# hirofumi0810/tensorflow_end2end_speech_recognition

Hardware: AMD Instinct MI355X
Metric: acoustic frames/sec (train), TIMIT-shaped BLSTM-CTC (higher is better)
Workload: dtype bf16; 1 GPU; TIMIT 61-phone 5x256 BLSTM-CTC, B=16/GPU, D=120, C=62, seq_len~U{100..778}, dropout 0.2, rmsprop, train step; global_batch=16, parallelism=dp1, padded_to=own Tmax per rank

## Files before the change

### include/asr_hip.h

```cpp
#ifndef ASR_HIP_H_
#define ASR_HIP_H_

#include <stddef.h>
#include <stdint.h>

#ifdef __cplusplus
extern "C" {
#endif

typedef struct asr_handle asr_handle;
typedef void* asr_stream;

typedef enum {
  ASR_OK = 0,
  ASR_ERR_INVALID_ARG = -1,
  ASR_ERR_UNSUPPORTED = -2,
  ASR_ERR_HIP = -3,
  ASR_ERR_WORKSPACE = -4
} asr_status;

typedef enum { ASR_F32 = 0, ASR_BF16 = 1 } asr_dtype;

typedef enum {
  ASR_OPT_SGD = 0, ASR_OPT_MOMENTUM = 1, ASR_OPT_NESTEROV = 2, ASR_OPT_ADAGRAD = 3,
// ... 165 lines not shown
                    int Cout, int relu, int out_f32, void* out, asr_stream s);
int asr_conv3x4_bwd_data(asr_handle* h, const void* dy, int N, int H, int W, int Cout, const void* wt_bwd, int Cin,
                         float* dx, asr_stream s);
int asr_conv3x4_bwd_weight_bias(asr_handle* h, const void* x, const void* dy, int N, int H, int W, int Cin, int Cout,
                                float* dw, float* dbias, asr_stream s);
size_t asr_bn_workspace_bytes(long long M, int C);
int asr_bn_stats(asr_handle* h, const float* x, long long M, int C, float eps, float momentum, const float* avg_mean,
                 const float* avg_var, float* stats, void* ws, asr_stream s);
int asr_bn_apply(asr_handle* h, int out_dtype, const float* x, int N, int H, int W, int C, const float* mean,
                 const float* var, const float* gamma, const float* beta, float eps, int pool, void* out,
                 uint8_t* argmax, asr_stream s);
int asr_bn_bwd(asr_handle* h, int out_dtype, const float* dz, const uint8_t* argmax, int pool, const float* x, int N,
               int H, int W, int C, const float* stats, const float* gamma, int relu_gate, float* dgamma, float* dbeta,
               void* dx, void* ws, asr_stream s);
int asr_softmax_xent_soft(asr_handle* h, const float* logits, const float* targets, int rows, int C, float grad_scale,
                          float* row_loss, float* dlogits, asr_stream s);

int asr_lstm_prep_weights(asr_handle* h, int dtype, const float* kernel, const float* bias,
                          int Din, int H, void* wx_il, float* bias_il,
                          void* packed_fwd, void* packed_bwd, asr_stream s);
int asr_lstm_prep_layer(asr_handle* h, int dtype, int ndir, const float* const* vars, int Din, int ldk, int H,
                        void* wxT, void* wx_cat, float* bias_cat, void* packed_fwd, void* packed_bwd,
                        float* peep_out, asr_stream s);
int asr_lstm_grad_finish(asr_handle* h, int ndir, float* const* grads, int rows, int H, const float* dw_il,
                         const float* dpeep_dbias, int has_peep, asr_stream s);
int asr_gate_deinterleave(asr_handle* h, const float* in, int ld_in, float* out, int ld_out,
                          int rows, int H, asr_stream s);

int asr_lstm_fwd(asr_handle* h, int dtype, int T, int B, int H, int ndir,
                 const float* xproj, const void* wh_packed, const float* peep,
                 const int32_t* seq_len, float forget_bias, float cell_clip,
                 void* gates, void* hout, float* cs, float* c_final, float* h_final,
                 asr_stream s);

int asr_lstm_bwd(asr_handle* h, int dtype, int T, int B, int H, int ndir,
                 const float* dhout, const void* gates, const float* cs,
                 const void* wh_packed_bwd, const float* peep, const int32_t* seq_len,
                 const float* d_c_final, const float* d_h_final,
                 void* dgates, float* dpeep_dbias, float* dpeep_workspace, asr_stream s);
int asr_lstm_bwd_ex(asr_handle* h, int dtype, int T, int B, int H, int ndir,
                    const float* dhout, const void* gates, const float* cs,
                    const void* wh_packed_bwd, const float* peep, const int32_t* seq_len,
                    const float* d_c_final, const float* d_h_final, float clip_no_grad,
                    void* dgates, float* dpeep_dbias, float* dpeep_workspace, asr_stream s);

int asr_check_async_errors(asr_handle* h, unsigned* flags_out);
// ... 443 lines not shown
```

### tensorflow_end2end_speech_recognition_amd/_lib.py

```python
import ctypes as C
import os

_PKG = os.path.dirname(os.path.abspath(__file__))
LIB_PATH = os.path.join(_PKG, 'libasr_hip.so')

ASR_F32, ASR_BF16 = 0, 1
OPTIMIZER_IDS = {'sgd': 0, 'momentum': 1, 'nestrov': 2, 'adagrad': 3, 'adadelta': 4,
                 'rmsprop': 5, 'adam': 6}

_vp, _i, _f, _sz = C.c_void_p, C.c_int, C.c_float, C.c_size_t
_i64, _u64 = C.c_int64, C.c_uint64

SIGNATURES = {
    'asr_abi_version': (_i, []),
    'asr_create': (_i, [C.POINTER(_vp), _i]),
    'asr_create_ex': (_i, [C.POINTER(_vp), _i, _sz]),
    'asr_scratch_bytes': (_sz, [_vp]),
    'asr_destroy': (_i, [_vp]),
    'asr_set_xcd_skip': (_i, [_vp, _i]),
    'asr_set_gemm_tn_workgroups': (_i, [_vp, _i]),
    'asr_last_error_string': (C.c_char_p, [_vp]),
    'asr_device_info': (_i, [_vp, C.POINTER(_i), C.c_char_p, _i]),
    'asr_bt_to_tb': (_i, [_vp, _i, _vp, _vp, _i, _i, _i, _vp]),
    'asr_bt_to_tb_ld': (_i, [_vp, _i, _vp, _vp, _i, _i, _i, _i, _vp]),
    'asr_transpose2d': (_i, [_vp, _i, _vp, _i, _i, _i, _vp, _i, _vp]),
    'asr_cast_from_f32': (_i, [_vp, _i, _vp, _vp, _sz, _vp]),
    'asr_cast_to_f32': (_i, [_vp, _i, _vp, _vp, _sz, _vp]),
    'asr_apply_mask': (_i, [_vp, _i, _vp, _vp, _vp, _sz, _vp]),
    'asr_dropout_mask': (_i, [_vp, _vp, _sz, _f, _u64, _u64, _vp]),
    'asr_touch': (_i, [_vp, _vp, _sz, _vp]),
    'asr_dropout_apply': (_i, [_vp, _i, _vp, _vp, _sz, _f, _u64, _u64, _vp]),
    'asr_relu_bwd_drop': (_i, [_vp, _i, _vp, _vp, _sz, _f, _u64, _u64, _vp, _vp]),
    'asr_colsum': (_i, [_vp, _i, _vp, _i, _i, _i, _vp, _vp]),
    'asr_gemm': (_i, [_vp, _i, _i, _i, _i, _i, _i, _i, _vp, _i, _vp, _i, _vp, _i, _vp, _i, _vp]),
# ... 22 lines not shown
    'asr_relu_bwd_scaled': (_i, [_vp, _i, _vp, _vp, _sz, _f, _vp, _vp]),
    'asr_maxpool2x2_bwd': (_i, [_vp, _vp, _vp, _i, _i, _i, _i, _vp, _vp]),
    'asr_relu_bwd': (_i, [_vp, _i, _vp, _vp, _vp, _sz, _vp, _vp]),
    'asr_maxpool2x2_relu_bwd': (_i, [_vp, _i, _vp, _vp, _vp, _i, _i, _i, _i, _vp, _f, _u64, _u64, _i, _vp]),
    'asr_conv3x5_prep_weights': (_i, [_vp, _vp, _i, _i, _vp, _vp, _vp]),
    'asr_conv3x5_fwd': (_i, [_vp, _vp, _i, _i, _i, _i, _vp, _vp, _i, _i, _vp, _vp]),
    'asr_conv3x5_fwd_drop': (_i, [_vp, _vp, _i, _i, _i, _i, _vp, _vp, _i, _f, _u64, _u64, _vp, _vp]),
    'asr_conv3x5_bwd_data': (_i, [_vp, _vp, _i, _i, _i, _i, _vp, _i, _vp, _vp]),
    'asr_conv3x5_bwd_data_relu': (_i, [_vp, _vp, _i, _i, _i, _i, _vp, _i, _vp, _f, _u64, _u64, _i, _vp, _vp]),
    'asr_conv3x5_bwd_weight_bias': (_i, [_vp, _vp, _vp, _i, _i, _i, _i, _i, _vp, _vp, _vp]),
    'asr_maxpool3x1_fwd': (_i, [_vp, _i, _vp, _i, _i, _i, _i, _vp, _vp, _f, _u64, _u64, _i, _vp]),
    'asr_maxpool3x1_bwd': (_i, [_vp, _i, _vp, _vp, _i, _i, _i, _i, _vp, _vp]),
    'asr_conv3x4_prep_weights': (_i, [_vp, _vp, _i, _i, _vp, _vp, _vp]),
    'asr_conv3x4_fwd': (_i, [_vp, _vp, _i, _i, _i, _i, _vp, _vp, _i, _i, _i, _vp, _vp]),
    'asr_conv3x4_bwd_data': (_i, [_vp, _vp, _i, _i, _i, _i, _vp, _i, _vp, _vp]),
    'asr_conv3x4_bwd_weight_bias': (_i, [_vp, _vp, _vp, _i, _i, _i, _i, _i, _vp, _vp, _vp]),
    'asr_bn_workspace_bytes': (_sz, [_i64, _i]),
    'asr_bn_stats': (_i, [_vp, _vp, _i64, _i, _f, _f, _vp, _vp, _vp, _vp, _vp]),
    'asr_bn_apply': (_i, [_vp, _i, _vp, _i, _i, _i, _i, _vp, _vp, _vp, _vp, _f, _i, _vp, _vp, _vp]),
    'asr_bn_bwd': (_i, [_vp, _i, _vp, _vp, _i, _vp, _i, _i, _i, _i, _vp, _vp, _i, _vp, _vp, _vp, _vp, _vp]),
    'asr_softmax_xent_soft': (_i, [_vp, _vp, _vp, _i, _i, _f, _vp, _vp, _vp]),
    'asr_lstm_prep_weights': (_i, [_vp, _i, _vp, _vp, _i, _i, _vp, _vp, _vp, _vp, _vp]),
    'asr_lstm_prep_layer': (_i, [_vp, _i, _i, _vp, _i, _i, _i, _vp, _vp, _vp, _vp, _vp, _vp, _vp]),
    'asr_lstm_grad_finish': (_i, [_vp, _i, _vp, _i, _i, _vp, _vp, _i, _vp]),
    'asr_gate_deinterleave': (_i, [_vp, _vp, _i, _vp, _i, _i, _i, _vp]),
    'asr_lstm_fwd': (_i, [_vp, _i, _i, _i, _i, _i, _vp, _vp, _vp, _vp, _f, _f, _vp, _vp, _vp, _vp, _vp, _vp]),
    'asr_lstm_bwd': (_i, [_vp, _i, _i, _i, _i, _i, _vp, _vp, _vp, _vp, _vp, _vp, _vp, _vp, _vp, _vp,
                          _vp, _vp]),
    'asr_lstm_bwd_ex': (_i, [_vp, _i, _i, _i, _i, _i, _vp, _vp, _vp, _vp, _vp, _vp, _vp, _vp, _f, _vp, _vp,
                             _vp, _vp]),
    'asr_gru_fwd': (_i, [_vp, _i, _i, _i, _i, _vp, _vp, _vp, _vp, _vp, _i, _vp, _vp, _vp, _vp, _vp, _vp, _vp]),
    'asr_gru_bwd': (_i, [_vp, _i, _i, _i, _i, _vp, _vp, _vp, _vp, _vp, _vp, _vp, _vp, _vp, _i, _vp, _vp, _vp, _vp]),
    'asr_check_async_errors': (_i, [_vp, C.POINTER(C.c_uint)]),
    'asr_peek_async_errors': (_i, [_vp, _vp, _vp]),
    'asr_clear_async_errors': (_i, [_vp, _vp]),
    'asr_debug_set_lstm_flags': (_i, [_i]),
    'asr_debug_set_gru_persistent': (_i, [_i]),
    'asr_cluster_tile_groups': (_i, [_i, _i, _i, _i, C.POINTER(_i), C.POINTER(_i), _i]),
    'asr_recurrence_path_counts': (_i, [_vp, C.POINTER(C.c_ulonglong)]),
    'asr_reset_recurrence_path_counts': (_i, [_vp]),
    'asr_gru_kernel_counts': (_i, [_vp, C.POINTER(C.c_ulonglong)]),
    'asr_reset_gru_kernel_counts': (_i, [_vp]),
    'asr_lstm_kernel_counts': (_i, [_vp, C.POINTER(C.c_ulonglong), _i]),
    'asr_reset_lstm_kernel_counts': (_i, [_vp]),
    'asr_att_path_counts': (_i, [_vp, C.POINTER(C.c_ulonglong), _i]),
    'asr_reset_att_path_counts': (_i, [_vp]),
# ... 214 lines not shown
```

### tensorflow_end2end_speech_recognition_amd/csrc/lstm.hip

```cpp
#include "common.h"
#include <stdlib.h>

namespace {

template <typename T> struct LT;
template <> struct LT<float> {
  static constexpr int KV = 16;
  static constexpr int PAD = 4;
  typedef f32x4_t g4_t;
  static __device__ __forceinline__ g4_t pack(float a, float b, float c, float d) { return (g4_t){a, b, c, d}; }
  static __device__ __forceinline__ void unpack(const g4_t& v, float& a, float& b, float& c, float& d) {
    a = v[0]; b = v[1]; c = v[2]; d = v[3];
  }
  static __device__ __forceinline__ float cvt(float v) { return v; }
};
typedef __attribute__((ext_vector_type(4))) __bf16 bf16x4_t;
template <> struct LT<bf16_t> {
  static constexpr int KV = 32;
  static constexpr int PAD = 8;
  typedef bf16x4_t g4_t;
  static __device__ __forceinline__ g4_t pack(float a, float b, float c, float d) {
    return (g4_t){(__bf16)a, (__bf16)b, (__bf16)c, (__bf16)d};
  }
  static __device__ __forceinline__ void unpack(const g4_t& v, float& a, float& b, float& c, float& d) {
// ... 103 lines not shown
        const int k = ks * KV + kin;
        pf[(size_t)d * n_wh + i2] = Elem<T>::from_f32(wh[(size_t)k * G + q * H + ub * 16 + n]);
      }
      {
        const int KS = G / KV;
        const int ks = frag % KS;
        const int ub = frag / KS;
        const int kp = ks * KV + kin;
        pb[(size_t)d * n_wh + i2] = Elem<T>::from_f32(wh[(size_t)(ub * 16 + n) * G + (kp & 3) * H + (kp >> 2)]);
      }
      continue;
    }
    idx -= n_wh;
    if (idx < (size_t)G) {
      const int cp = (int)idx;
      bias_cat[(size_t)d * G + cp] = v.bias[d][(cp & 3) * H + (cp >> 2)];
      continue;
    }
    idx -= G;
    peep_out[(size_t)d * 3 * H + idx] = v.peep[d][idx / H][idx % H];
  }
}

struct GradVars { float* kernel[2]; float* bias[2]; float* peep[2][3]; };
__global__ void grad_finish_kernel(GradVars v, int ndir, int R, int H, const float* __restrict__ dw_il,
                                   const float* __restrict__ dpeep, int has_peep) {
  const int G = 4 * H;
  const size_t n_w = (size_t)R * G;
  const size_t per_dir = n_w + G + (has_peep ? (size_t)3 * H : 0);
  for (size_t gidx = blockIdx.x * (size_t)blockDim.x + threadIdx.x; gidx < per_dir * ndir;
       gidx += (size_t)gridDim.x * blockDim.x) {
    const int d = (int)(gidx / per_dir);
    size_t idx = gidx - (size_t)d * per_dir;
    if (idx < n_w) {
      const int r = (int)(idx / G), c = (int)(idx % G);
      const int q = c / H, j = c % H;
      v.kernel[d][idx] = dw_il[(size_t)d * n_w + (size_t)r * G + j * 4 + q];
      continue;
    }
    idx -= n_w;
    if (idx < (size_t)G) {
      v.bias[d][idx] = dpeep[((size_t)d * 7 + 3) * H + idx];
      continue;
    }
    idx -= G;
    v.peep[d][idx / H][idx % H] = dpeep[(size_t)d * 7 * H + idx];
// ... 559 lines not shown
    ASR_FAIL(h, ASR_ERR_INVALID_ARG, "asr_lstm_prep_layer: bad args (H=%d must be a multiple of 64, ldk=%d >= Din=%d)", H, ldk, Din);
  PrepVars v;
  memset(&v, 0, sizeof(v));
  for (int d = 0; d < ndir; ++d) {
    v.kernel[d] = vars[d * 5 + 0];
    v.bias[d] = vars[d * 5 + 1];
    for (int k = 0; k < 3; ++k) v.peep[d][k] = vars[d * 5 + 2 + k];
    if (!v.kernel[d] || !v.bias[d]) ASR_FAIL(h, ASR_ERR_INVALID_ARG, "asr_lstm_prep_layer: kernel / bias of direction %d missing", d);
    if (peep_out && (!v.peep[d][0] || !v.peep[d][1] || !v.peep[d][2]))
      ASR_FAIL(h, ASR_ERR_INVALID_ARG, "asr_lstm_prep_layer: peep_out given but a peephole vector of direction %d is missing", d);
  }
  const size_t total = (size_t)ndir * ((size_t)4 * H * ldk + (size_t)(Din + H + 1) * 4 * H + (peep_out ? 3 * H : 0));
  const int blocks = (int)((total + 255) / 256 < 4096 ? (total + 255) / 256 : 4096);
  if (dtype == ASR_F32)
    hipLaunchKernelGGL(prep_layer_kernel<float>, dim3(blocks), dim3(256), 0, (hipStream_t)s, v, ndir, Din, ldk, H,
                       (float*)wxT, (float*)wx_cat, bias_cat, (float*)packed_fwd, (float*)packed_bwd, peep_out);
  else
    hipLaunchKernelGGL(prep_layer_kernel<bf16_t>, dim3(blocks), dim3(256), 0, (hipStream_t)s, v, ndir, Din, ldk, H,
                       (bf16_t*)wxT, (bf16_t*)wx_cat, bias_cat, (bf16_t*)packed_fwd, (bf16_t*)packed_bwd, peep_out);
  ASR_CHECK_LAUNCH(h, "asr_lstm_prep_layer");
  return ASR_OK;
}

extern "C" int asr_lstm_grad_finish(asr_handle* h, int ndir, float* const* grads, int rows, int H,
                                    const float* dw_il, const float* dpeep_dbias, int has_peep, asr_stream s) {
  if (!h) return ASR_ERR_INVALID_ARG;
  if ((ndir != 1 && ndir != 2) || !grads || !dw_il || !dpeep_dbias || rows <= 0 || H <= 0)
    ASR_FAIL(h, ASR_ERR_INVALID_ARG, "asr_lstm_grad_finish: bad args");
  GradVars v;
  memset(&v, 0, sizeof(v));
  for (int d = 0; d < ndir; ++d) {
    v.kernel[d] = grads[d * 5 + 0];
    v.bias[d] = grads[d * 5 + 1];
    for (int k = 0; k < 3; ++k) v.peep[d][k] = grads[d * 5 + 2 + k];
    if (!v.kernel[d] || !v.bias[d] || (has_peep && (!v.peep[d][0] || !v.peep[d][1] || !v.peep[d][2])))
      ASR_FAIL(h, ASR_ERR_INVALID_ARG, "asr_lstm_grad_finish: a gradient pointer of direction %d is missing", d);
  }
  const size_t total = (size_t)ndir * ((size_t)(rows + 1) * 4 * H + (has_peep ? 3 * H : 0));
  const int blocks = (int)((total + 255) / 256 < 4096 ? (total + 255) / 256 : 4096);
  hipLaunchKernelGGL(grad_finish_kernel, dim3(blocks), dim3(256), 0, (hipStream_t)s, v, ndir, rows, H, dw_il,
                     dpeep_dbias, has_peep);
  ASR_CHECK_LAUNCH(h, "asr_lstm_grad_finish");
  return ASR_OK;
}

extern "C" int asr_lstm_fwd(asr_handle* h, int dtype, int T, int B, int H, int ndir,
// ... 105 lines not shown
```

### tensorflow_end2end_speech_recognition_amd/models/ctc/ctc.py

```python
import os as _os

import numpy as np
import torch

from ... import ops
from ..._lib import ASR_BF16, ASR_F32
from ...utils.io.labels.sparsetensor import dense_to_flat, sparse_to_flat
from ...utils.evaluation.edit_distance import compute_ler as _ler
from ...utils.parameter import ParamStore
from ..encoders.core.residual import check_residual, load_residual
from ..encoders.core.subsample import check_subsample, load_subsampled, shift_lengths
from ..encoders.load_encoder import load
from ..model_base import ModelBase


def truncated_normal(rng, stddev, shape):
    x = rng.normal(0.0, stddev, size=shape)
    bad = np.abs(x) > 2 * stddev
    while bad.any():
        x[bad] = rng.normal(0.0, stddev, size=int(bad.sum()))
        bad = np.abs(x) > 2 * stddev
    return x


# ... 67 lines not shown
        self.seed = seed

        self.bottleneck_dim = int(bottleneck_dim) if bottleneck_dim not in (None, 0) else None
        self.subsample_list = check_subsample(subsample_list, subsample_type, num_layers)
        self.subsample_type = subsample_type
        if any(self.subsample_list):
            load_subsampled(encoder_type)
        self.encoder_skip = check_residual(encoder_residual, encoder_dense_residual)
        if self.encoder_skip is not None:
            load_residual(encoder_type)
            if any(self.subsample_list):
                raise ValueError('skip connections join layers of one frame rate: not with a true subsample_list entry')
            if num_layers < 2:
                self.encoder_skip = None

        self.encoder = self._create_encoder(encoder_type, input_size, splice, num_stack, num_units, num_layers,
                                            lstm_impl, use_peephole, parameter_init, clip_activation)

        rng = np.random.RandomState(seed)
        self.store = ParamStore(self.device)
        enc_dim = self.encoder.build(self.store, input_size * num_stack * splice, rng)
        self._enc_dim = enc_dim
        self._head_imgs = None
        self._head_state = None
        self._declare_heads(rng, enc_dim, parameter_init)
        self.store.finalize()
        self._tape = None

    def _create_encoder(self, encoder_type, input_size, splice, num_stack, num_units, num_layers, lstm_impl,
                        use_peephole, parameter_init, clip_activation):
        if encoder_type in ['blstm', 'lstm']:
            if any(self.subsample_list):
                return load_subsampled(encoder_type)(
                    num_units=num_units, num_proj=self.num_proj, num_layers=num_layers,
                    lstm_impl=lstm_impl, use_peephole=use_peephole, parameter_init=parameter_init,
                    clip_activation=clip_activation, time_major=True, dtype=self._requested_dtype,
                    subsample_list=self.subsample_list, subsample_type=self.subsample_type)
            if self.encoder_skip is not None:
                return load_residual(encoder_type)(
                    num_units=num_units, num_proj=self.num_proj, num_layers=num_layers,
                    lstm_impl=lstm_impl, use_peephole=use_peephole, parameter_init=parameter_init,
                    clip_activation=clip_activation, time_major=True, dtype=self._requested_dtype,
                    dense=self.encoder_skip == 'dense')
            return load(encoder_type)(
                num_units=num_units, num_proj=self.num_proj, num_layers=num_layers,
                lstm_impl=lstm_impl, use_peephole=use_peephole, parameter_init=parameter_init,
# ... 68 lines not shown
            self._bn = None
            self._head_in = x_op
            return logits
        enc = x_op
        self._bn = None
        if self.bottleneck_dim:
            h = ops.gemm(x_op.view(T * Bp, E), sh['bottleneck/weights'], bias=self.store['bottleneck/biases'],
                         relu=True)
            mask = None
            hd = h
            if rng_state is not None:
                mask = ops.dropout_mask(h.shape, float(keep_prob), rng_state[0] + 11, rng_state[1], enc.device)
                hd = ops.apply_mask(h, mask)
            self._bn = dict(x=x_op, h=h, hd=hd, mask=mask)
            x_op, E = hd.view(T, Bp, self.bottleneck_dim), self.bottleneck_dim
        self._head_in = x_op
        logits = torch.empty((T, Bp, self.num_classes), dtype=torch.float32, device=enc.device)
        ops.gemm(x_op.view(T * Bp, E), sh[self.head_scope + '/weights'], bias=self.store[self.head_scope + '/biases'],
                 out=logits.view(T * Bp, self.num_classes))
        return logits

    def _refresh_head_shadow(self):
        if getattr(self, '_want_head_imgs', False):
            ops.ctc_head_prep(self.store[self.head_scope + '/weights'], out=self._head_imgs)
        sh = self.store.shadow(self.dtype)
        if sh is not self.store:
            for n in self.store.names:
                if n.endswith('/weights') and not n.startswith(('VGG', 'CNN', 'bridge', 'fc')):
                    sh[n]

    def _enc_operand(self):
        return self.encoder._out_op

    def create_placeholders(self):
        self.inputs_pl_list.append(Placeholder('input', np.float32,
                                               [None, None, self.input_size * self.num_stack * self.splice]))
        self.labels_pl_list.append(Placeholder('labels'))
        self.inputs_seq_len_pl_list.append(Placeholder('inputs_seq_len', np.int32, [None]))
        self.keep_prob_pl_list.append(Placeholder('keep_prob', np.float32))

    @staticmethod
    def _labels_to_flat(labels, batch_size):
        if isinstance(labels, (list, tuple)) and len(labels) == 3 and np.asarray(labels[0]).ndim == 2 \
                and np.asarray(labels[0]).shape[1] == 2 and np.asarray(labels[2]).shape == (2,):
            return sparse_to_flat(labels, batch_size)
        if torch.is_tensor(labels):
            labels = labels.cpu().numpy()
# ... 162 lines not shown
```

### tensorflow_end2end_speech_recognition_amd/models/encoders/core/blstm.py

```python
import collections
import os as _os

import numpy as np
import torch

from .... import ops
from ...._lib import ASR_F32
from ....utils.parameter import ParamStore
from . import rnn_util
from .rnn_util import LSTMLayer, LSTMPLayer, declare_lstm_vars, declare_lstmp_vars

WARM_BPTT = _os.environ.get('ASR_WARM_BPTT', '1') != '0'
ENC_HALVES = _os.environ.get('ASR_ENC_HALVES', '0') == '1'
PIPE_LANE = 6

LSTMStateTuple = collections.namedtuple('LSTMStateTuple', ('c', 'h'))

LSTM_IMPLS = ('BasicLSTMCell', 'LSTMCell', 'LSTMBlockCell', 'LSTMBlockFusedCell', 'CudnnLSTM')


class _RecurrentEncoderBase(object):
    ndir = 2
    scope_fmt = 'blstm_hidden%d'

    def __init__(self, num_units, num_proj, num_layers, lstm_impl, use_peephole, parameter_init,
                 clip_activation, time_major=True, name='lstm_encoder', dtype=ASR_F32, seed=0):
        assert num_proj != 0
        if lstm_impl not in LSTM_IMPLS:
            raise IndexError('lstm_impl is "BasicLSTMCell" or "LSTMCell" or "LSTMBlockCell" or '
                             '"LSTMBlockFusedCell" or "CudnnLSTM".')
        self.num_units = num_units
        self.num_proj = num_proj if lstm_impl == 'LSTMCell' else None
        if self.num_proj is not None and type(self).__name__ not in ('BLSTMEncoder', 'LSTMEncoder', 'VGGBLSTMEncoder',
                                                                     'VGGLSTMEncoder', 'MultitaskBLSTMEncoder',
                                                                     'MultitaskLSTMEncoder', 'CLDNNEncoder'):
            raise ValueError('LSTMCell projection layers (num_proj) are implemented for the blstm / lstm / vgg_* / '
# ... 4 lines not shown
        self.parameter_init = parameter_init
        self.clip_activation = None if lstm_impl == 'BasicLSTMCell' else clip_activation
        self.time_major = time_major
        self.name = name
        self.dtype = ops.dtype_id(dtype)
        self.layer_dtype = self.dtype
        if self.num_proj is not None:
            self.dtype = ASR_F32
        self.seed = seed
        self.layers = None
        self.store = None
        self.scope_prefix = ''
        self.num_layers_sub = None
        self.grad_ready_hook = None
        self.side_extra = None
        self.side_extra_event = None
        self.defer_top_dropout = False
        self._top_deferred, self._top_drop = False, None
        self.want_f32_outputs = True
        self.halves = ENC_HALVES
        self.layers_b = None
        self._split = 0
        self._rows = None

    def build(self, store, input_dim, rng, scope_prefix=''):
        self.store = store
        self.scope_prefix = scope_prefix
        self.layers = []
        din = input_dim
        H = self.num_units
        if self.num_proj is not None:
            P = int(self.num_proj)
            for i in range(1, self.num_layers + 1):
                bases = self._declare_projected(store, i, din, P, rng)
                self.layers.append(LSTMPLayer(store, bases, din, H, P, self.use_peephole, 1.0, self.clip_activation,
                                              dtype=self.layer_dtype))
                din = self.ndir * P
            self.output_dim = self.ndir * P
            return self.output_dim
        for i in range(1, self.num_layers + 1):
            bases = self._declare(store, i, din, rng)
            self.layers.append(LSTMLayer(store, bases, din, H, self.use_peephole, 1.0,
                                         self.clip_activation))
            din = self.ndir * H
        self.output_dim = self.ndir * H
        return self.output_dim
# ... 18 lines not shown
        self._ensure_built(inputs)
        lens_host = getattr(self, '_lens_host', None)
        self._lens_host = None
        if self.num_proj is not None:
            return self._call_projected(inputs, inputs_seq_len, keep_prob, is_training, drop_masks, rng_state)
        B, T, _ = inputs.shape
        self.pad_b = (-B) % 16
        if self.pad_b:
            inputs = torch.cat([inputs, inputs.new_zeros(self.pad_b, T, inputs.shape[2])], 0)
            inputs_seq_len = torch.cat([inputs_seq_len, inputs_seq_len.new_zeros(self.pad_b)], 0)
        self.batch = B
        seq_len = inputs_seq_len.to(torch.int32).contiguous()
        Tt, Bp = T, inputs.shape[0]
        D = inputs.shape[2]
        ldk0 = (D + 63) // 64 * 64 if self.dtype != ASR_F32 else D

        if rng_state is None and drop_masks is None and is_training and keep_prob is not None and keep_prob < 1.0:
            self._dropout_calls = getattr(self, '_dropout_calls', 0) + 1
            rng_state = (self.seed, self._dropout_calls << 40)

        def rs_of(li):
            return (rng_state[0], rng_state[1] + li * (1 << 32)) if rng_state is not None else None

        preps, ready_w, ready_m = [], [], []
        with ops.side_lane(inputs.device):
            fold = self.side_extra is not None and len(self.layers) >= 2
            self.side_extra_event = None
            for li, layer in enumerate(self.layers):
                preps.append(layer.prepare(inputs.device, self.dtype, Tt, Bp, 1.0, False, None, None,
                                           ldk=ldk0 if li == 0 else None))
                if fold and li + 1 == len(self.layers):
                    self.side_extra()
                ready_w.append(ops.stream_event())
            if self.side_extra is not None and not fold:
                self.side_extra()
                self.side_extra_event = ops.stream_event()
            for li, layer in enumerate(self.layers):
                dm = drop_masks[li] if drop_masks is not None else None
                preps[li]['mask'] = layer.make_mask(inputs.device, Tt, Bp, keep_prob, is_training, rs_of(li), dm)
                ready_m.append(ops.stream_event())
        self._split = self._split_rows(Bp) if drop_masks is None else 0
        self._top_deferred, self._top_drop = False, None
        plans = rnn_util.row_plans(lens_host, B, Tt, Bp, self._split) if (self.dtype != ASR_F32 and inputs.is_cuda) \
            else None
        self._rows = None
        if plans is not None:
            self._rows = [(t, int(p.size)) for t, p in zip(ops.upload_ints(inputs.device, plans), plans)]
        if self._split:
            x, finals = self._forward_halves(inputs, seq_len, preps, ready_w, ready_m, keep_prob, is_training, ldk0)
            return self._finish_call(x, finals, seq_len, B)
        x = ops.bt_to_tb(inputs.contiguous(), self.dtype, ld=ldk0)
        final = None
        finals = []
        for li, layer in enumerate(self.layers):
            if not rnn_util.FORK_ONCE or li == 0:
                ops.wait_event(ready_w[li])
            elif li == 1:
                ops.wait_event(ready_w[-1])
            top = li + 1 == len(self.layers)
            mk = preps[li]['mask']
            defer = top and self.defer_top_dropout and self.num_layers_sub is None and (mk is None or isinstance(mk, tuple))
            x, final = layer.forward(x, seq_len, self.dtype, keep_prob, is_training, prep=preps[li],
                                     mask_event=ready_m[li], rows=self._rows[0] if self._rows else None,
                                     defer_mask=defer or self._connects(li))
            if defer:
                self._top_deferred, self._top_drop = True, mk
            x = self._connect(li, x, mk, seq_len)
            finals.append(final)
            if self.num_layers_sub is not None and li + 1 == self.num_layers_sub:
                self._out_sub_op, self._final_sub_ch = x, final
        return self._finish_call(x, finals, seq_len, B)

    def _connects(self, li):
        return False

    def _connect(self, li, x, mask, seq_len):
        return x

    def _finish_call(self, x, finals, seq_len, B):
        self.seq_len_padded = seq_len
        self._out_op = x
        out = ops.cast_to_f32(x) if (x.dtype != torch.float32 and self.want_f32_outputs) else x
        self._out_tm = out
        cf, hf = finals[-1]
        self._final_ch = (cf, hf)
        self._finals = finals
        final_state = self._state_tuple(finals, len(finals))
        out_user = out[:, :B]
        if not self.time_major:
            out_user = out_user.transpose(0, 1)
        return out_user, final_state

    def _split_rows(self, Bp):
        tiles = Bp // 16
# ... 185 lines not shown
```

### tensorflow_end2end_speech_recognition_amd/ops.py

```python
import ctypes as C
import math
import os
import time as _time

import numpy as np
import torch

from . import _lib
from ._lib import ASR_BF16, ASR_F32

TORCH_DTYPE = {ASR_F32: torch.float32, ASR_BF16: torch.bfloat16}


def dtype_id(dtype):
    if dtype in (ASR_F32, 'f32', 'fp32', 'float32', torch.float32):
        return ASR_F32
    if dtype in (ASR_BF16, 'bf16', 'bfloat16', torch.bfloat16):
        return ASR_BF16
    raise ValueError('dtype must be f32 or bf16, got %r' % (dtype,))


_lane = 0
_side = {}

# ... 937 lines not shown
                   pb=torch.empty((H * 4 * H,), dtype=tdt, device=dev))
    h.check(h.lib.asr_lstm_prep_weights(h.h, dtype, _p(kernel), _p(bias), din, H, _p(out['wx_il']),
                                        _p(out['bias_il']), _p(out['pf']), _p(out['pb']), _s()),
            'asr_lstm_prep_weights')
    return out


def gate_deinterleave(src, dst, H):
    h = _h(src)
    h.check(h.lib.asr_gate_deinterleave(h.h, C.c_void_p(src.data_ptr()), src.stride(0),
                                        C.c_void_p(dst.data_ptr()), dst.stride(0), src.shape[0], H, _s()),
            'asr_gate_deinterleave')
    return dst


def _ptr_table(rows):
    flat = []
    for r in rows:
        r = list(r) + [None] * (5 - len(r))
        flat.extend(t.data_ptr() if t is not None else None for t in r)
    return (C.c_void_p * len(flat))(*flat)


def lstm_prep_layer(variables, din, H, dtype, ldk=None):
    k0 = variables[0][0]
    h = _h(k0)
    ndir = len(variables)
    ldk = din if ldk is None else int(ldk)
    for v in variables:
        _chk(v[0], torch.float32, 'kernel')
        if v[0].shape != (din + H, 4 * H):
            raise ValueError('kernel must be [Din+H,4H]')
    has_peep = len(variables[0]) >= 5 and variables[0][2] is not None
    dev, tdt = k0.device, TORCH_DTYPE[dtype]
    out = dict(wxT=torch.empty((ndir * 4 * H, ldk), dtype=tdt, device=dev),
               wx_cat=torch.empty((din, ndir * 4 * H), dtype=tdt, device=dev),
               bias=torch.empty((ndir * 4 * H,), dtype=torch.float32, device=dev),
               whf=torch.empty((ndir, H * 4 * H), dtype=tdt, device=dev),
               whb=torch.empty((ndir, H * 4 * H), dtype=tdt, device=dev),
               peep=torch.empty((ndir, 3, H), dtype=torch.float32, device=dev) if has_peep else None)
    h.check(h.lib.asr_lstm_prep_layer(h.h, dtype, ndir, _ptr_table(variables), din, ldk, H, _p(out['wxT']),
                                      _p(out['wx_cat']), _p(out['bias']), _p(out['whf']), _p(out['whb']),
                                      _p(out['peep']), _s()), 'asr_lstm_prep_layer')
    return out


def lstm_grad_finish(grads, dw_il, dpeep, H):
    h = _h(dw_il)
    ndir, rows, _ = dw_il.shape
    has_peep = len(grads[0]) >= 5 and grads[0][2] is not None
    h.check(h.lib.asr_lstm_grad_finish(h.h, ndir, _ptr_table(grads), rows, H, _p(dw_il), _p(dpeep),
                                       1 if has_peep else 0, _s()), 'asr_lstm_grad_finish')


LSTM_UNITS = (64, 128, 192, 256, 320, 512)


def lstm_units_supported(H):
    return int(H) in LSTM_UNITS


def lstm_fwd(xproj, wh_packed, peep, seq_len, H, ndir, dtype, forget_bias=1.0, cell_clip=0.0,
             want_final=True):
    h = _h(xproj)
    _chk(xproj, torch.float32, 'xproj')
    _chk(seq_len, torch.int32, 'seq_len')
    T, B, G = xproj.shape
# ... 2000 lines not shown
```

### tensorflow_end2end_speech_recognition_amd/utils/parameter.py

```python
import numpy as np
import torch

from .. import ops
from .._lib import ASR_BF16


class ParamStore(object):
    def __init__(self, device):
        self.device = device
        self._specs = []
        self._index = {}
        self.flat = None
        self.grad = None
        self.views = {}
        self.gviews = {}
        self.finalized = False
        self._shadow = None
        self._shadow_dirty = True
        self._backup = None
        self.perturbed = False

    def declare(self, name, shape, init):
        if self.finalized:
            raise RuntimeError('ParamStore already finalized; cannot declare %s' % name)
        if name in self._index:
            raise ValueError('variable %s already exists' % name)
        init = np.asarray(init, dtype=np.float32).reshape(shape)
        self._index[name] = len(self._specs)
        self._specs.append((name, tuple(int(s) for s in shape), init))

    def finalize(self):
        offs = [0]
        starts = []
        pos = 0
        for name, shape, _ in self._specs:
            n = int(np.prod(shape)) if len(shape) else 1
            starts.append(pos)
            pos += (n + 15) // 16 * 16
            offs.append(pos)
        self.total = pos
        host = np.zeros(self.total, dtype=np.float32)
        for (name, shape, init), st in zip(self._specs, starts):
            host[st:st + init.size] = init.ravel()
# ... 11 lines not shown
        self.finalized = True
        self._shadow_dirty = True

    def __getitem__(self, name):
        return self.views[name]

    def g(self, name):
        return self.gviews[name]

    def bucket(self, first, last):
        i0, i1 = self._index[first], self._index[last]
        if i1 < i0:
            raise ValueError('bucket: %s is declared after %s' % (first, last))
        off = self.offsets_host[i0:i1 + 2] - self.offsets_host[i0]
        start, end = int(self.offsets_host[i0]), int(self.offsets_host[i1 + 1])
        return dict(start=start, end=end, names=self.names[i0:i1 + 1], grad=self.grad[start:end],
                    plan=ops.ClipPlan(off, self.flat.device))

    def num_params(self):
        return int(sum(int(np.prod(s[1])) if len(s[1]) else 1 for s in self._specs))

    def mark_dirty(self):
        self._shadow_dirty = True

    def shadow(self, dtype):
        if dtype != ASR_BF16:
            return self
        if self._shadow is None:
            self._shadow = _Shadow(self)
        if self._shadow_dirty:
            self._shadow.invalidate()
            self._shadow_dirty = False
        return self._shadow

    def perturb(self, std, seed, offset):
        if self.perturbed:
            raise RuntimeError('ParamStore.perturb: the previous perturbation was not restored')
        if self._backup is None:
            self._backup = torch.empty_like(self.flat)
        ops.weight_noise_perturb(self.flat, self._backup, std, seed, offset)
        self.perturbed = True
        self.mark_dirty()

    def restore(self):
        if not self.perturbed:
            return
# ... 95 lines not shown
```

Measured before the change: 766,000 frames/s.

## Batch LSTM weight prep into one multi-layer kernel and cache images by version

Adds a grouped prep kernel that packs the input, recurrent and bias/peephole weight images for all LSTM layers in a single launch instead of one launch per layer on a side stream. The encoder now caches these prepared images and the CTC head image, keyed on the parameter store's tensor version and a mutation epoch, so they are rebuilt only when the weights change. In training the optimizer updates the weights every step, so each step still runs one fused prep call, issued on the main stream rather than overlapped on the side lane. This trades the removed launches and side-stream events for losing that overlap, and adds key-tracking complexity.

```diff
diff --git a/include/asr_hip.h b/include/asr_hip.h
--- a/include/asr_hip.h
+++ b/include/asr_hip.h
@@ -211,6 +211,16 @@
 int asr_lstm_prep_layer(asr_handle* h, int dtype, int ndir, const float* const* vars, int Din, int ldk, int H,
                         void* wxT, void* wx_cat, float* bias_cat, void* packed_fwd, void* packed_bwd,
                         float* peep_out, asr_stream s);
+typedef struct asr_lstm_prep_desc {
+  int ndir;
+  const float* const* vars;
+  int Din, ldk, H;
+  void *wxT, *wx_cat;
+  float* bias_cat;
+  void *packed_fwd, *packed_bwd;
+  float* peep_out;
+} asr_lstm_prep_desc;
+int asr_lstm_prep_layers(asr_handle* h, int dtype, int nlayers, const asr_lstm_prep_desc* layers, asr_stream s);
 int asr_lstm_grad_finish(asr_handle* h, int ndir, float* const* grads, int rows, int H, const float* dw_il,
                          const float* dpeep_dbias, int has_peep, asr_stream s);
 int asr_gate_deinterleave(asr_handle* h, const float* in, int ld_in, float* out, int ld_out,
diff --git a/tensorflow_end2end_speech_recognition_amd/_lib.py b/tensorflow_end2end_speech_recognition_amd/_lib.py
--- a/tensorflow_end2end_speech_recognition_amd/_lib.py
+++ b/tensorflow_end2end_speech_recognition_amd/_lib.py
@@ -10,6 +10,11 @@
 
 _vp, _i, _f, _sz = C.c_void_p, C.c_int, C.c_float, C.c_size_t
 _i64, _u64 = C.c_int64, C.c_uint64
+
+class LstmPrepDesc(C.Structure):
+    _fields_ = [('ndir', _i), ('vars', _vp), ('Din', _i), ('ldk', _i), ('H', _i), ('wxT', _vp), ('wx_cat', _vp),
+                ('bias_cat', _vp), ('packed_fwd', _vp), ('packed_bwd', _vp), ('peep_out', _vp)]
+
 
 SIGNATURES = {
     'asr_abi_version': (_i, []),
@@ -78,6 +83,7 @@
     'asr_softmax_xent_soft': (_i, [_vp, _vp, _vp, _i, _i, _f, _vp, _vp, _vp]),
     'asr_lstm_prep_weights': (_i, [_vp, _i, _vp, _vp, _i, _i, _vp, _vp, _vp, _vp, _vp]),
     'asr_lstm_prep_layer': (_i, [_vp, _i, _i, _vp, _i, _i, _i, _vp, _vp, _vp, _vp, _vp, _vp, _vp]),
+    'asr_lstm_prep_layers': (_i, [_vp, _i, _i, _vp, _vp]),
     'asr_lstm_grad_finish': (_i, [_vp, _i, _vp, _i, _i, _vp, _vp, _i, _vp]),
     'asr_gate_deinterleave': (_i, [_vp, _vp, _i, _vp, _i, _i, _i, _vp]),
     'asr_lstm_fwd': (_i, [_vp, _i, _i, _i, _i, _i, _vp, _vp, _vp, _vp, _f, _f, _vp, _vp, _vp, _vp, _vp, _vp]),
diff --git a/tensorflow_end2end_speech_recognition_amd/csrc/lstm.hip b/tensorflow_end2end_speech_recognition_amd/csrc/lstm.hip
--- a/tensorflow_end2end_speech_recognition_amd/csrc/lstm.hip
+++ b/tensorflow_end2end_speech_recognition_amd/csrc/lstm.hip
@@ -149,6 +149,109 @@
   }
 }
 
+constexpr int PREP_MAX_LAYERS = 16;
+struct PrepLayer {
+  PrepVars v;
+  void *wxT, *wx_cat;
+  float* bias_cat;
+  void *pf, *pb;
+  float* peep_out;
+  int ndir, Din, ldk, H;
+  int block0, upd, nX, nB, nF;
+};
+struct PrepGroup { PrepLayer l[PREP_MAX_LAYERS]; int n; };
+static_assert(sizeof(PrepGroup) <= 4096, "PrepGroup must fit the kernel argument segment");
+
+template <typename T>
+__global__ __launch_bounds__(256) void prep_layers_kernel(PrepGroup g) {
+  constexpr int KV = LT<T>::KV;
+  constexpr int E = 16 / sizeof(T);
+  static_assert(KV == 4 * E, "a fragment is four row groups of E elements");
+  constexpr int SX = 129, SB = 136, SF = 40;
+  __shared__ float tile[32 * SX];
+  int li = 0;
+  while (li + 1 < g.n && (int)blockIdx.x >= g.l[li + 1].block0) ++li;
+  const PrepLayer& L = g.l[li];
+  const int H = L.H, G = 4 * H, Din = L.Din, ldk = L.ldk, ndir = L.ndir, HT = H / 32;
+  int u = (int)blockIdx.x - L.block0;
+  const int d = u / L.upd;
+  u -= d * L.upd;
+  const float* __restrict__ kernel = L.v.kernel[d];
+  const float* __restrict__ wh = kernel + (size_t)Din * G;
+  const size_t n_wh = (size_t)H * G;
+  const int t = threadIdx.x;
+  if (u < L.nX) {
+    const int r0 = (u / HT) * 32, j0 = (u % HT) * 32;
+#pragma unroll
+    for (int i = 0; i < 16; ++i) {
+      const int e = t + 256 * i, rl = e >> 7, c = e & 127, q = c >> 5, jj = c & 31, r = r0 + rl;
+      tile[rl * SX + jj * 4 + q] = r < Din ? kernel[(size_t)r * G + q * H + j0 + jj] : 0.f;
+    }
+    __syncthreads();
+    T* __restrict__ wx_cat = (T*)L.wx_cat;
+    T* __restrict__ wxT = (T*)L.wxT;
+#pragma unroll
+    for (int i = 0; i < 16; ++i) {
+      const int e = t + 256 * i, rl = e >> 7, cpl = e & 127, r = r0 + rl;
+      if (r < Din) wx_cat[(size_t)r * ndir * G + (size_t)d * G + j0 * 4 + cpl] = Elem<T>::from_f32(tile[rl * SX + cpl]);
+    }
+#pragma unroll
+    for (int i = 0; i < 16; ++i) {
+      const int e = t + 256 * i, cpl = e >> 5, rl = e & 31, r = r0 + rl;
+      if (r < ldk) wxT[((size_t)d * G + j0 * 4 + cpl) * ldk + r] = Elem<T>::from_f32(tile[rl * SX + cpl]);
+    }
+    return;
+  }
+  u -= L.nX;
+  if (u < L.nB) {
+    const int ub = u / HT, j0 = (u % HT) * 32;
+#pragma unroll
+    for (int i = 0; i < 8; ++i) {
+      const int e = t + 256 * i, n = e >> 7, c = e & 127, q = c >> 5, jj = c & 31;
+      tile[n * SB + jj * 4 + q] = wh[(size_t)(ub * 16 + n) * G + q * H + j0 + jj];
+    }
+    __syncthreads();
+    T* __restrict__ pb = (T*)L.pb + (size_t)d * n_wh + (size_t)ub * 16 * G + (size_t)64 * j0;
+#pragma unroll
+    for (int i = 0; i < 8; ++i) {
+      const int o = t + 256 * i, e = o % E, n = (o / E) & 15, rg = (o / (16 * E)) & 3, ksl = o / (64 * E);
+      pb[o] = Elem<T>::from_f32(tile[n * SB + ksl * KV + rg * E + e]);
+    }
+    return;
+  }
+  u -= L.nB;
+  if (u < L.nF) {
+    const int k0 = (u / (4 * HT)) * 32, q = (u % (4 * HT)) / HT, u0 = (u % HT) * 32;
+#pragma unroll
+    for (int i = 0; i < 4; ++i) {
+      const int e = t + 256 * i, kl = e >> 5, cl = e & 31;
+      tile[kl * SF + cl] = wh[(size_t)(k0 + kl) * G + q * H + u0 + cl];
+    }
+    __syncthreads();
+    T* __restrict__ pf = (T*)L.pf + (size_t)d * n_wh;
+#pragma unroll
+    for (int i = 0; i < 4; ++i) {
+      const int o4 = t + 256 * i, ubl = o4 >> 9, o = o4 & 511;
+      const int e = o % E, n = (o / E) & 15, rg = (o / (16 * E)) & 3, ksl = o / (64 * E);
+      const int ub = u0 / 16 + ubl, kl = ksl * KV + rg * E + e;
+      pf[((size_t)(ub * 4 + q) * H + k0) * 16 + o] = Elem<T>::from_f32(tile[kl * SF + ubl * 16 + n]);
+    }
+    return;
+  }
+  u -= L.nF;
+  if (u < G / 256) {
+    const int cp = u * 256 + t;
+    L.bias_cat[(size_t)d * G + cp] = L.v.bias[d][(cp & 3) * H + (cp >> 2)];
+    return;
+  }
+  const int idx = (u - G / 256) * 256 + t;
+  if (idx < 3 * H) {
+    const int k = idx / H;
+    const float* p = k == 0 ? L.v.peep[d][0] : k == 1 ? L.v.peep[d][1] : L.v.peep[d][2];
+    L.peep_out[(size_t)d * 3 * H + idx] = p[idx - k * H];
+  }
+}
+
 struct GradVars { float* kernel[2]; float* bias[2]; float* peep[2][3]; };
 __global__ void grad_finish_kernel(GradVars v, int ndir, int R, int H, const float* __restrict__ dw_il,
                                    const float* __restrict__ dpeep, int has_peep) {
@@ -754,6 +857,57 @@
   return ASR_OK;
 }
 
+extern "C" int asr_lstm_prep_layers(asr_handle* h, int dtype, int nlayers, const asr_lstm_prep_desc* layers,
+                                    asr_stream s) {
+  if (!h) return ASR_ERR_INVALID_ARG;
+  if (!asr_dtype_ok(dtype) || nlayers < 0 || (nlayers && !layers))
+    ASR_FAIL(h, ASR_ERR_INVALID_ARG, "asr_lstm_prep_layers: bad args");
+  for (int i = 0; i < nlayers; ++i) {
+    const asr_lstm_prep_desc& L = layers[i];
+    if ((L.ndir != 1 && L.ndir != 2) || !L.vars || !L.wxT || !L.wx_cat || !L.bias_cat || !L.packed_fwd ||
+        !L.packed_bwd || L.Din <= 0 || L.ldk < L.Din || L.H <= 0 || L.H % 64)
+      ASR_FAIL(h, ASR_ERR_INVALID_ARG, "asr_lstm_prep_layers: layer %d: H=%d must be a multiple of 64, ldk=%d >= Din=%d", i,
+               L.H, L.ldk, L.Din);
+    for (int d = 0; d < L.ndir; ++d) {
+      if (!L.vars[d * 5] || !L.vars[d * 5 + 1])
+        ASR_FAIL(h, ASR_ERR_INVALID_ARG, "asr_lstm_prep_layers: kernel / bias of layer %d, direction %d missing", i, d);
+      if (L.peep_out && (!L.vars[d * 5 + 2] || !L.vars[d * 5 + 3] || !L.vars[d * 5 + 4]))
+        ASR_FAIL(h, ASR_ERR_INVALID_ARG, "asr_lstm_prep_layers: peep_out given but a peephole vector of layer %d, direction %d is missing", i, d);
+    }
+  }
+  for (int i0 = 0; i0 < nlayers; i0 += PREP_MAX_LAYERS) {
+    PrepGroup g;
+    memset(&g, 0, sizeof(g));
+    g.n = nlayers - i0 < PREP_MAX_LAYERS ? nlayers - i0 : PREP_MAX_LAYERS;
+    long long blocks = 0;
+    for (int i = 0; i < g.n; ++i) {
+      const asr_lstm_prep_desc& L = layers[i0 + i];
+      PrepLayer& P = g.l[i];
+      for (int d = 0; d < L.ndir; ++d) {
+        P.v.kernel[d] = L.vars[d * 5 + 0];
+        P.v.bias[d] = L.vars[d * 5 + 1];
+        for (int k = 0; k < 3; ++k) P.v.peep[d][k] = L.vars[d * 5 + 2 + k];
+      }
+      P.wxT = L.wxT, P.wx_cat = L.wx_cat, P.bias_cat = L.bias_cat, P.pf = L.packed_fwd, P.pb = L.packed_bwd;
+      P.peep_out = L.peep_out;
+      P.ndir = L.ndir, P.Din = L.Din, P.ldk = L.ldk, P.H = L.H;
+      const long long HT = L.H / 32;
+      const long long nX = ((long long)L.ldk + 31) / 32 * HT, nB = (L.H / 16) * HT, nF = HT * HT * 4;
+      const long long upd = nX + nB + nF + 4 * L.H / 256 + (L.peep_out ? (3 * L.H + 255) / 256 : 0);
+      if (blocks + L.ndir * upd > 0x7fffffffLL)
+        ASR_FAIL(h, ASR_ERR_INVALID_ARG, "asr_lstm_prep_layers: layer %d: too many units for one grid", i0 + i);
+      P.block0 = (int)blocks, P.upd = (int)upd, P.nX = (int)nX, P.nB = (int)nB, P.nF = (int)nF;
+      blocks += L.ndir * upd;
+    }
+    if (dtype == ASR_F32)
+      hipLaunchKernelGGL(prep_layers_kernel<float>, dim3((unsigned)blocks), dim3(256), 0, (hipStream_t)s, g);
+    else
+      hipLaunchKernelGGL(prep_layers_kernel<bf16_t>, dim3((unsigned)blocks), dim3(256), 0, (hipStream_t)s, g);
+    ASR_CHECK_LAUNCH(h, "asr_lstm_prep_layers");
+  }
+  return ASR_OK;
+}
+
 extern "C" int asr_lstm_grad_finish(asr_handle* h, int ndir, float* const* grads, int rows, int H,
                                     const float* dw_il, const float* dpeep_dbias, int has_peep, asr_stream s) {
   if (!h) return ASR_ERR_INVALID_ARG;
diff --git a/tensorflow_end2end_speech_recognition_amd/models/ctc/ctc.py b/tensorflow_end2end_speech_recognition_amd/models/ctc/ctc.py
--- a/tensorflow_end2end_speech_recognition_amd/models/ctc/ctc.py
+++ b/tensorflow_end2end_speech_recognition_amd/models/ctc/ctc.py
@@ -113,6 +113,7 @@
         enc_dim = self.encoder.build(self.store, input_size * num_stack * splice, rng)
         self._enc_dim = enc_dim
         self._head_imgs = None
+        self._head_key = None
         self._head_state = None
         self._declare_heads(rng, enc_dim, parameter_init)
         self.store.finalize()
@@ -227,7 +228,10 @@
 
     def _refresh_head_shadow(self):
         if getattr(self, '_want_head_imgs', False):
-            ops.ctc_head_prep(self.store[self.head_scope + '/weights'], out=self._head_imgs)
+            key = self.store.image_key() if getattr(self.encoder, 'weight_images', False) else None
+            if key is None or key != self._head_key:
+                ops.ctc_head_prep(self.store[self.head_scope + '/weights'], out=self._head_imgs)
+                self._head_key = key
         sh = self.store.shadow(self.dtype)
         if sh is not self.store:
             for n in self.store.names:
diff --git a/tensorflow_end2end_speech_recognition_amd/models/encoders/core/blstm.py b/tensorflow_end2end_speech_recognition_amd/models/encoders/core/blstm.py
--- a/tensorflow_end2end_speech_recognition_amd/models/encoders/core/blstm.py
+++ b/tensorflow_end2end_speech_recognition_amd/models/encoders/core/blstm.py
@@ -12,6 +12,7 @@
 
 WARM_BPTT = _os.environ.get('ASR_WARM_BPTT', '1') != '0'
 ENC_HALVES = _os.environ.get('ASR_ENC_HALVES', '0') == '1'
+WEIGHT_IMAGES = _os.environ.get('ASR_WEIGHT_IMAGES', '1') != '0'
 PIPE_LANE = 6
 
 LSTMStateTuple = collections.namedtuple('LSTMStateTuple', ('c', 'h'))
@@ -62,6 +63,8 @@
         self.layers_b = None
         self._split = 0
         self._rows = None
+        self.weight_images = WEIGHT_IMAGES
+        self._images, self._image_key = None, None
 
     def build(self, store, input_dim, rng, scope_prefix=''):
         self.store = store
@@ -126,23 +129,12 @@
         def rs_of(li):
             return (rng_state[0], rng_state[1] + li * (1 << 32)) if rng_state is not None else None
 
-        preps, ready_w, ready_m = [], [], []
-        with ops.side_lane(inputs.device):
-            fold = self.side_extra is not None and len(self.layers) >= 2
-            self.side_extra_event = None
-            for li, layer in enumerate(self.layers):
-                preps.append(layer.prepare(inputs.device, self.dtype, Tt, Bp, 1.0, False, None, None,
-                                           ldk=ldk0 if li == 0 else None))
-                if fold and li + 1 == len(self.layers):
-                    self.side_extra()
-                ready_w.append(ops.stream_event())
-            if self.side_extra is not None and not fold:
-                self.side_extra()
-                self.side_extra_event = ops.stream_event()
-            for li, layer in enumerate(self.layers):
-                dm = drop_masks[li] if drop_masks is not None else None
-                preps[li]['mask'] = layer.make_mask(inputs.device, Tt, Bp, keep_prob, is_training, rs_of(li), dm)
-                ready_m.append(ops.stream_event())
+        if self.weight_images:
+            preps, ready_w, ready_m = self._cached_preps(inputs.device, ldk0, Tt, Bp, keep_prob, is_training, rs_of,
+                                                         drop_masks)
+        else:
+            preps, ready_w, ready_m = self._side_preps(inputs.device, ldk0, Tt, Bp, keep_prob, is_training, rs_of,
+                                                       drop_masks)
         self._split = self._split_rows(Bp) if drop_masks is None else 0
         self._top_deferred, self._top_drop = False, None
         plans = rnn_util.row_plans(lens_host, B, Tt, Bp, self._split) if (self.dtype != ASR_F32 and inputs.is_cuda) \
@@ -174,6 +166,45 @@
             if self.num_layers_sub is not None and li + 1 == self.num_layers_sub:
                 self._out_sub_op, self._final_sub_ch = x, final
         return self._finish_call(x, finals, seq_len, B)
+
+    def _cached_preps(self, device, ldk0, Tt, Bp, keep_prob, is_training, rs_of, drop_masks):
+        key = self.store.image_key() + (self.dtype, ldk0)
+        if key != self._image_key:
+            self._images = ops.lstm_prep_layers(
+                [dict(variables=layer._vars(self.store.__getitem__), din=layer.din, H=layer.H, dtype=self.dtype,
+                      ldk=ldk0 if li == 0 else None) for li, layer in enumerate(self.layers)])
+            self._image_key = key
+        self.side_extra_event = None
+        if self.side_extra is not None:
+            self.side_extra()
+        preps, ready_m = [], []
+        for li, layer in enumerate(self.layers):
+            dm = drop_masks[li] if drop_masks is not None else None
+            w = dict(self._images[li])
+            w['mask'] = layer.make_mask(device, Tt, Bp, keep_prob, is_training, rs_of(li), dm)
+            preps.append(w)
+            ready_m.append(ops.stream_event() if torch.is_tensor(w['mask']) and w['mask'].is_cuda else None)
+        return preps, [None] * len(self.layers), ready_m
+
+    def _side_preps(self, device, ldk0, Tt, Bp, keep_prob, is_training, rs_of, drop_masks):
+        preps, ready_w, ready_m = [], [], []
+        with ops.side_lane(device):
+            fold = self.side_extra is not None and len(self.layers) >= 2
+            self.side_extra_event = None
+            for li, layer in enumerate(self.layers):
+                preps.append(layer.prepare(device, self.dtype, Tt, Bp, 1.0, False, None, None,
+                                           ldk=ldk0 if li == 0 else None))
+                if fold and li + 1 == len(self.layers):
+                    self.side_extra()
+                ready_w.append(ops.stream_event())
+            if self.side_extra is not None and not fold:
+                self.side_extra()
+                self.side_extra_event = ops.stream_event()
+            for li, layer in enumerate(self.layers):
+                dm = drop_masks[li] if drop_masks is not None else None
+                preps[li]['mask'] = layer.make_mask(device, Tt, Bp, keep_prob, is_training, rs_of(li), dm)
+                ready_m.append(ops.stream_event())
+        return preps, ready_w, ready_m
 
     def _connects(self, li):
         return False
diff --git a/tensorflow_end2end_speech_recognition_amd/ops.py b/tensorflow_end2end_speech_recognition_amd/ops.py
--- a/tensorflow_end2end_speech_recognition_amd/ops.py
+++ b/tensorflow_end2end_speech_recognition_amd/ops.py
@@ -983,9 +983,8 @@
     return (C.c_void_p * len(flat))(*flat)
 
 
-def lstm_prep_layer(variables, din, H, dtype, ldk=None):
+def _prep_layer_args(variables, din, H, dtype, ldk, out=None):
     k0 = variables[0][0]
-    h = _h(k0)
     ndir = len(variables)
     ldk = din if ldk is None else int(ldk)
     for v in variables:
@@ -994,16 +993,105 @@
             raise ValueError('kernel must be [Din+H,4H]')
     has_peep = len(variables[0]) >= 5 and variables[0][2] is not None
     dev, tdt = k0.device, TORCH_DTYPE[dtype]
-    out = dict(wxT=torch.empty((ndir * 4 * H, ldk), dtype=tdt, device=dev),
-               wx_cat=torch.empty((din, ndir * 4 * H), dtype=tdt, device=dev),
-               bias=torch.empty((ndir * 4 * H,), dtype=torch.float32, device=dev),
-               whf=torch.empty((ndir, H * 4 * H), dtype=tdt, device=dev),
-               whb=torch.empty((ndir, H * 4 * H), dtype=tdt, device=dev),
-               peep=torch.empty((ndir, 3, H), dtype=torch.float32, device=dev) if has_peep else None)
+    shapes = dict(wxT=((ndir * 4 * H, ldk), tdt), wx_cat=((din, ndir * 4 * H), tdt),
+                  bias=((ndir * 4 * H,), torch.float32), whf=((ndir, H * 4 * H), tdt), whb=((ndir, H * 4 * H), tdt),
+                  peep=((ndir, 3, H), torch.float32))
+    if out is None:
+        out = dict((k, torch.empty(sh, dtype=dt, device=dev)) for k, (sh, dt) in shapes.items())
+        if not has_peep:
+            out['peep'] = None
+    else:
+        for k, (sh, dt) in shapes.items():
+            t = out.get(k)
+            if k == 'peep' and not has_peep:
+                if t is not None:
+                    raise ValueError('lstm_prep_layers: out has a peephole image for a layer without peepholes')
+                continue
+            if t is None or tuple(t.shape) != sh or t.dtype != dt or t.device != dev or not t.is_contiguous():
+                raise ValueError('lstm_prep_layers: out[%r] must be a contiguous %s tensor of shape %s on %s'
+                                 % (k, dt, sh, dev))
+    return ndir, ldk, out
+
+
+def lstm_prep_layer(variables, din, H, dtype, ldk=None):
+    h = _h(variables[0][0])
+    ndir, ldk, out = _prep_layer_args(variables, din, H, dtype, ldk)
     h.check(h.lib.asr_lstm_prep_layer(h.h, dtype, ndir, _ptr_table(variables), din, ldk, H, _p(out['wxT']),
                                       _p(out['wx_cat']), _p(out['bias']), _p(out['whf']), _p(out['whb']),
                                       _p(out['peep']), _s()), 'asr_lstm_prep_layer')
-    return out
+    _count_prep(variables[0][0].device, per_layer=1)
+    return out
+
+
+_lstm_prep_layer_native = lstm_prep_layer
+_prep_counts = {}
+
+
+def _prep_key(device):
+    if isinstance(device, torch.device):
+        return (device.index or 0) if device.type == 'cuda' else -1
+    return -1 if device in ('cpu', None) else int(device)
+
+
+def _count_prep(device, grouped=0, per_layer=0):
+    c = _prep_counts.setdefault(_prep_key(device), [0, 0])
+    c[0] += grouped
+    c[1] += per_layer
+
+
+def prep_counts(device=0):
+    c = _prep_counts.get(_prep_key(device), (0, 0))
+    return dict(grouped=int(c[0]), per_layer=int(c[1]))
+
+
+def reset_prep_counts(device=0):
+    _prep_counts.pop(_prep_key(device), None)
+
+
+def lstm_prep_layers(specs, out=None):
+    specs = list(specs)
+    if out is not None and len(out) != len(specs):
+        raise ValueError('lstm_prep_layers: %d output dicts for %d layers' % (len(out), len(specs)))
+    if not specs:
+        return []
+    k0 = specs[0]['variables'][0][0]
+    if not k0.is_cuda:
+        per_layer = globals()['lstm_prep_layer']
+        if per_layer is _lstm_prep_layer_native:
+            _h(k0)
+        res = []
+        for i, sp in enumerate(specs):
+            w = per_layer(sp['variables'], sp['din'], sp['H'], sp['dtype'], ldk=sp.get('ldk'))
+            _count_prep(k0.device, per_layer=1)
+            if out is not None:
+                for k, t in w.items():
+                    if t is not None:
+                        out[i][k].copy_(t)
+                w = out[i]
+            res.append(w)
+        return res
+    h = _h(k0)
+    dtype = specs[0]['dtype']
+    descs = (_lib.LstmPrepDesc * len(specs))()
+    res, tables = [], []
+    for i, sp in enumerate(specs):
+        if sp['dtype'] != dtype:
+            raise ValueError('lstm_prep_layers: one operand dtype for all layers')
+        if sp['variables'][0][0].device != k0.device:
+            raise ValueError('lstm_prep_layers: all layers on one device')
+        ndir, ldk, o = _prep_layer_args(sp['variables'], sp['din'], sp['H'], dtype, sp.get('ldk'),
+                                        out[i] if out is not None else None)
+        tab = _ptr_table(sp['variables'])
+        tables.append(tab)
+        d = descs[i]
+        d.ndir, d.vars, d.Din, d.ldk, d.H = ndir, C.addressof(tab), sp['din'], ldk, sp['H']
+        d.wxT, d.wx_cat, d.bias_cat = o['wxT'].data_ptr(), o['wx_cat'].data_ptr(), o['bias'].data_ptr()
+        d.packed_fwd, d.packed_bwd = o['whf'].data_ptr(), o['whb'].data_ptr()
+        d.peep_out = o['peep'].data_ptr() if o.get('peep') is not None else None
+        res.append(o)
+    h.check(h.lib.asr_lstm_prep_layers(h.h, dtype, len(specs), C.addressof(descs), _s()), 'asr_lstm_prep_layers')
+    _count_prep(k0.device, grouped=(len(specs) + 15) // 16)
+    return res
 
 
 def lstm_grad_finish(grads, dw_il, dpeep, H):
diff --git a/tensorflow_end2end_speech_recognition_amd/utils/parameter.py b/tensorflow_end2end_speech_recognition_amd/utils/parameter.py
--- a/tensorflow_end2end_speech_recognition_amd/utils/parameter.py
+++ b/tensorflow_end2end_speech_recognition_amd/utils/parameter.py
@@ -19,6 +19,7 @@
         self._shadow_dirty = True
         self._backup = None
         self.perturbed = False
+        self.epoch = 0
 
     def declare(self, name, shape, init):
         if self.finalized:
@@ -76,6 +77,10 @@
 
     def mark_dirty(self):
         self._shadow_dirty = True
+        self.epoch += 1
+
+    def image_key(self):
+        return (self.flat._version, self.epoch)
 
     def shadow(self, dtype):
         if dtype != ASR_BF16:
```

Measured after the change: 774,300 frames/s (median of 6 runs). 1.01x the previous value.
